# NTHU-LSALAB/KubeShare

Hardware: AMD Instinct MI355X
Metric: aggregate images/sec, co-located shared-GPU pods (higher is better)
Workload: dtype bf16; 1 GPU; model=resnet50, global_batch=512, image_size=224, parallelism=2 pods @ request=0.5, 2/GPU, pods_per_gpu=2, miopen_find=False, lease_accounting=sampled-busy

## Files before the change

kubeshare_amd/models/resnet.py:

```python
from __future__ import annotations

import torch
import torch.nn as nn

from .pool import FusedMaxPool2d


class Bottleneck(nn.Module):
    expansion = 4
    fused_ops = False

    def __init__(self, in_ch: int, width: int, stride: int = 1):
        super().__init__()
        out_ch = width * self.expansion
        self.conv1 = nn.Conv2d(in_ch, width, 1, bias=False)
        self.bn1 = nn.BatchNorm2d(width)
        self.conv2 = nn.Conv2d(width, width, 3, stride=stride, padding=1,
                               bias=False)
        self.bn2 = nn.BatchNorm2d(width)
        self.conv3 = nn.Conv2d(width, out_ch, 1, bias=False)
        self.bn3 = nn.BatchNorm2d(out_ch)
        self.relu = nn.ReLU(inplace=True)
        self.down = None
        if stride != 1 or in_ch != out_ch:
            self.down = nn.Sequential(
                nn.Conv2d(in_ch, out_ch, 1, stride=stride, bias=False),
                nn.BatchNorm2d(out_ch),
            )

    def forward(self, x):
        if self.fused_ops:
            from .. import ops
            identity = x if self.down is None else \
                ops.bn_relu(self.down[0](x), self.down[1], relu=False)
            out = ops.bn_relu(self.conv1(x), self.bn1)
            out = ops.bn_relu(self.conv2(out), self.bn2)
            return ops.bn_relu(self.conv3(out), self.bn3, res=identity)
        identity = x if self.down is None else self.down(x)
        out = self.relu(self.bn1(self.conv1(x)))
        out = self.relu(self.bn2(self.conv2(out)))
        out = self.bn3(self.conv3(out))
        return self.relu(out + identity)


class BasicBlock(nn.Module):
    expansion = 1
    fused_ops = False

    def __init__(self, in_ch: int, width: int, stride: int = 1):
        super().__init__()
        self.conv1 = nn.Conv2d(in_ch, width, 3, stride=stride, padding=1,
                               bias=False)
        self.bn1 = nn.BatchNorm2d(width)
        self.conv2 = nn.Conv2d(width, width, 3, padding=1, bias=False)
        self.bn2 = nn.BatchNorm2d(width)
        self.relu = nn.ReLU(inplace=True)
        self.down = None
        if stride != 1 or in_ch != width:
            self.down = nn.Sequential(
                nn.Conv2d(in_ch, width, 1, stride=stride, bias=False),
                nn.BatchNorm2d(width),
            )

    def forward(self, x):
        if self.fused_ops:
            from .. import ops
            identity = x if self.down is None else \
                ops.bn_relu(self.down[0](x), self.down[1], relu=False)
            out = ops.bn_relu(self.conv1(x), self.bn1)
            return ops.bn_relu(self.conv2(out), self.bn2, res=identity)
        identity = x if self.down is None else self.down(x)
        out = self.relu(self.bn1(self.conv1(x)))
        out = self.bn2(self.conv2(out))
        return self.relu(out + identity)


class ResNet(nn.Module):
    fused_ops = False

    def __init__(self, block, layers, num_classes: int = 1000):
        super().__init__()
        self.in_ch = 64
        self.conv1 = nn.Conv2d(3, 64, 7, stride=2, padding=3, bias=False)
        self.bn1 = nn.BatchNorm2d(64)
        self.relu = nn.ReLU(inplace=True)
        self.maxpool = FusedMaxPool2d(3, stride=2, padding=1)
        self.layer1 = self._make_layer(block, 64, layers[0])
        self.layer2 = self._make_layer(block, 128, layers[1], stride=2)
        self.layer3 = self._make_layer(block, 256, layers[2], stride=2)
        self.layer4 = self._make_layer(block, 512, layers[3], stride=2)
        self.avgpool = nn.AdaptiveAvgPool2d(1)
        self.fc = nn.Linear(512 * block.expansion, num_classes)
        for m in self.modules():
            if isinstance(m, nn.Conv2d):
                nn.init.kaiming_normal_(m.weight, mode="fan_out",
                                        nonlinearity="relu")
            elif isinstance(m, nn.BatchNorm2d):
                nn.init.ones_(m.weight)
                nn.init.zeros_(m.bias)

    def _make_layer(self, block, width, n, stride=1):
        layers = [block(self.in_ch, width, stride)]
        self.in_ch = width * block.expansion
        layers += [block(self.in_ch, width) for _ in range(n - 1)]
        return nn.Sequential(*layers)

    def forward(self, x):
        if self.fused_ops:
            from .. import ops
            x = self.maxpool(ops.bn_relu(self.conv1(x), self.bn1))
        else:
            x = self.maxpool(self.relu(self.bn1(self.conv1(x))))
        x = self.layer4(self.layer3(self.layer2(self.layer1(x))))
        x = torch.flatten(self.avgpool(x), 1)
        return self.fc(x)


def resnet18(num_classes: int = 1000) -> ResNet:
    return ResNet(BasicBlock, [2, 2, 2, 2], num_classes)


def resnet50(num_classes: int = 1000) -> ResNet:
    return ResNet(Bottleneck, [3, 4, 6, 3], num_classes)
```

kubeshare_amd/ops/__init__.py:

```python
from __future__ import annotations

import os

_HERE = os.path.dirname(os.path.abspath(__file__))
_BUILD_DIR = os.path.join(_HERE, "_build")
_SRCS = [os.path.join(_HERE, "hip", "ks_ops.hip"),
         os.path.join(_HERE, "hip", "bn_relu.hip"),
         os.path.join(_HERE, "hip", "pool.hip")]

_ext = None


def build_extension(verbose: bool = False):
    import torch
    from torch.utils import cpp_extension

    os.environ.setdefault("PYTORCH_ROCM_ARCH", "gfx950")
    os.makedirs(_BUILD_DIR, exist_ok=True)
    return cpp_extension.load(
        name="ks_ops",
        sources=_SRCS,
        build_directory=_BUILD_DIR,
        extra_cflags=["-O3"],
        verbose=verbose,
        is_python_module=True,
    )


def _load():
    global _ext
    if _ext is not None:
        return _ext
    import torch

    so = os.path.join(_BUILD_DIR, "ks_ops.so")
    if os.path.exists(so):
        import importlib.util

        spec = importlib.util.spec_from_file_location("ks_ops", so)
        mod = importlib.util.module_from_spec(spec)
        spec.loader.exec_module(mod)
        _ext = mod
        return _ext
    if torch.cuda.is_available():
        _ext = build_extension()
        return _ext
    raise ImportError(
        "kubeshare_amd.ops extension not built; run __graft_entry__.build()")


def burn(ms: float, blocks: int = 1024, threads: int = 256):
    _load().burn(float(ms), blocks, threads)


class FusedSGD:

    def __init__(self, params, lr: float, momentum: float = 0.9,
                 weight_decay: float = 0.0, graph_mode: str = "auto"):
        import torch

        self.params = [p for p in params if p.requires_grad]
        self.lr = lr
        self.momentum = momentum
        self.weight_decay = weight_decay
        self.momenta = [torch.zeros_like(p) for p in self.params]
        self._first = True
        self._graph_mode = graph_mode
        self._step_graph = None
        self._zero_graph = None
        self._graph_ptrs = None

    def _graphable(self):
        import torch
        if self._graph_mode == "off" or not torch.cuda.is_available():
            return False
        import os
        if os.environ.get("KUBESHARE_SGD_GRAPH", "1") == "0":
            return False
        return all(p.grad is not None and p.grad.is_cuda
                   for p in self.params)

    def zero_grad(self, set_to_none: bool = True):
        if self._zero_graph is not None and self._graph_ptrs == tuple(
                p.grad.data_ptr() if p.grad is not None else 0
                for p in self.params):
            self._zero_graph.replay()
            return
        for p in self.params:
            if p.grad is not None:
                if set_to_none and self._step_graph is None:
                    p.grad = None
                else:
                    p.grad.zero_()

    def _capture(self):
        import torch
        ext = _load()
        ps = [p.data for p in self.params]
        gs = [p.grad for p in self.params]
        vs = list(self.momenta)
        ptrs = tuple(g.data_ptr() for g in gs)
        step_g = torch.cuda.CUDAGraph()
        with torch.cuda.graph(step_g):
            ext.sgd_momentum_(ps, gs, vs, self.lr, self.momentum,
                              self.weight_decay)
        zero_g = torch.cuda.CUDAGraph()
        with torch.cuda.graph(zero_g):
            for g in gs:
                g.zero_()
        self._step_graph = step_g
        self._zero_graph = zero_g
        self._graph_ptrs = ptrs

    def step(self):
        ext = _load()
        if self._step_graph is not None and self._graph_ptrs == tuple(
                p.grad.data_ptr() if p.grad is not None else 0
                for p in self.params):
            self._step_graph.replay()
            return
        ps, gs, vs = [], [], []
        for p, v in zip(self.params, self.momenta):
            if p.grad is None:
                continue
            ps.append(p.data)
            gs.append(p.grad)
            vs.append(v)
        if self._first:
            self._first = False
        ext.sgd_momentum_(ps, gs, vs, self.lr, self.momentum,
                          self.weight_decay)
        if self._step_graph is None and self._graph_mode == "auto" and \
                len(gs) == len(self.params) and self._graphable():
            try:
                self._capture()
            except Exception:
                self._graph_mode = "off"


def _bn_relu_autograd():
    global _BNReLUFn
    if _BNReLUFn is not None:
        return _BNReLUFn
    import torch

    class BNReLUFn(torch.autograd.Function):

        @staticmethod
        def forward(ctx, x, res, weight, bias, running_mean, running_var,
                    training, momentum, eps, relu):
            ext = _load()
            w32 = weight.float()
            b32 = bias.float()
            if training:
                y, mean, invstd = ext.bn_relu_fwd_train(
                    x, w32, b32, running_mean, running_var, momentum, eps,
                    res, relu)
                ctx.save_for_backward(x, y, w32, b32, mean, invstd)
                ctx.with_res = res is not None
                ctx.relu = relu
                ctx.wdtype = weight.dtype
                return y
            y = ext.bn_relu_fwd_eval(x, w32, b32, running_mean.float(),
                                     running_var.float(), eps, res, relu)
            ctx.save_for_backward(x, y, w32, b32, running_mean.float(),
                                  (running_var.float() + eps).rsqrt())
            ctx.with_res = res is not None
            ctx.relu = relu
            ctx.wdtype = weight.dtype
            return y

        @staticmethod
        def backward(ctx, dy):
            ext = _load()
            x, y, w32, b32, mean, invstd = ctx.saved_tensors
            out = ext.bn_relu_bwd(x, y, dy, w32, b32, mean, invstd,
                                  ctx.with_res, ctx.relu)
            dx, dscale, dbias = out[0], out[1], out[2]
            dres = out[3] if ctx.with_res else None
            return (dx, dres, dscale.to(ctx.wdtype), dbias.to(ctx.wdtype),
                    None, None, None, None, None, None)

    _BNReLUFn = BNReLUFn
    return BNReLUFn


_BNReLUFn = None


def bn_relu(x, bn, res=None, relu=True):
    import torch

    supported = (x.dtype == torch.bfloat16 and x.size(1) % 8 == 0
                 and x.size(1) <= 2048 and x.is_cuda
                 and x.is_contiguous(memory_format=torch.channels_last))
    if supported and res is not None and res.dtype != torch.bfloat16:
        res = res.to(torch.bfloat16)
    if not supported:
        y = torch.nn.functional.batch_norm(
            x, bn.running_mean, bn.running_var, bn.weight, bn.bias,
            bn.training, bn.momentum, bn.eps)
        if res is not None:
            y = y + res
        return torch.relu(y) if relu else y
    if res is not None and not res.is_contiguous(
            memory_format=torch.channels_last):
        res = res.contiguous(memory_format=torch.channels_last)
    fn = _bn_relu_autograd()
    return fn.apply(x, res, bn.weight, bn.bias, bn.running_mean,
                    bn.running_var, bn.training, bn.momentum, bn.eps, relu)


_POOL_CONFIGS = ((3, 2, 1), (2, 2, 0))
_MaxPoolNHWCFn = None


def _pool_int(v):
    if type(v) is int:
        return v
    if isinstance(v, (tuple, list)) and len(v) == 2 and v[0] == v[1] \
            and type(v[0]) is int:
        return v[0]
    return None


def _pool_cfg(kernel_size, stride, padding):
    if stride is None or stride == () or stride == []:
        stride = kernel_size
    return (_pool_int(kernel_size), _pool_int(stride), _pool_int(padding))


def _pool_cfg_supported(x, cfg) -> bool:
    import torch

    if cfg not in _POOL_CONFIGS or x.dim() != 4:
        return False
    n, c, h, w = x.shape
    k, _, p = cfg
    return (x.is_cuda and x.dtype == torch.bfloat16
            and c % 8 == 0 and 8 <= c <= 2048 and n >= 1
            and h + 2 * p >= k and w + 2 * p >= k
            and n * h * w < 2 ** 31
            and x.is_contiguous(memory_format=torch.channels_last))


def fused_pool_enabled() -> bool:
    return os.environ.get("KUBESHARE_FUSED_POOL", "1") != "0"


def max_pool_supported(x, kernel_size, stride=None, padding=0) -> bool:
    return _pool_cfg_supported(x, _pool_cfg(kernel_size, stride, padding))


def _max_pool_autograd():
    global _MaxPoolNHWCFn
    if _MaxPoolNHWCFn is not None:
        return _MaxPoolNHWCFn
    import torch
    from torch.autograd.function import once_differentiable

    class MaxPoolNHWCFn(torch.autograd.Function):

        @staticmethod
        def forward(ctx, x, k, s, p, want_idx):
            out = _load().max_pool_nhwc_fwd(x, k, s, p, want_idx)
            if want_idx:
                ctx.save_for_backward(out[1])
                ctx.input_sizes = list(x.shape)
                ctx.cfg = (k, s, p)
            return out[0]

        @staticmethod
        @once_differentiable
        def backward(ctx, dy):
            (idx,) = ctx.saved_tensors
            if not dy.is_contiguous(memory_format=torch.channels_last):
                dy = dy.contiguous(memory_format=torch.channels_last)
            k, s, p = ctx.cfg
            dx = _load().max_pool_nhwc_bwd(dy, idx, ctx.input_sizes,
                                           k, s, p)
            return dx, None, None, None, None

    _MaxPoolNHWCFn = MaxPoolNHWCFn
    return MaxPoolNHWCFn


def max_pool_nhwc(x, kernel_size, stride=None, padding=0):
    import torch

    cfg = _pool_cfg(kernel_size, stride, padding)
    if not _pool_cfg_supported(x, cfg):
        return torch.nn.functional.max_pool2d(x, kernel_size, stride,
                                              padding)
# ... 12 lines not shown
```

kubeshare_amd/ops/hip/bn_relu.hip:

```cpp
#include <hip/hip_runtime.h>
#include <torch/extension.h>
#include <ATen/cuda/CUDAContext.h>

#include <vector>

typedef __attribute__((ext_vector_type(8))) unsigned short ushort8;
typedef __attribute__((ext_vector_type(8))) float float8;

__device__ __forceinline__ float bf16_to_f32(unsigned short u) {
  union {
    unsigned int i;
    float f;
  } v;
  v.i = ((unsigned int)u) << 16;
  return v.f;
}

__device__ __forceinline__ unsigned short f32_to_bf16(float f) {
  union {
    float f;
    unsigned int i;
  } v;
  v.f = f;
  unsigned int lsb = (v.i >> 16) & 1;
  v.i += 0x7fffu + lsb;
  return (unsigned short)(v.i >> 16);
}

#define KS_BN_BLOCK 512
#define KS_BN_UNROLL 4
#define KS_BN_UNROLL_STATS 8

__global__ void bn_stats_kernel(const ushort8* __restrict__ x,
                                float* __restrict__ part,
                                long long M, int CG) {
  __shared__ float s_red[KS_BN_BLOCK * 8];
  const int tid = threadIdx.x;
  const int cg = tid % CG;
  const int roff = tid / CG;
  const int rows_per_blk = KS_BN_BLOCK / CG;
  const bool active = roff < rows_per_blk;
  const long long stride = (long long)gridDim.x * rows_per_blk;

  float8 acc = {0, 0, 0, 0, 0, 0, 0, 0};
  float8 acc2 = {0, 0, 0, 0, 0, 0, 0, 0};
  long long row = active ? (long long)blockIdx.x * rows_per_blk + roff : M;
  for (; row + (KS_BN_UNROLL_STATS - 1) * stride < M;
       row += KS_BN_UNROLL_STATS * stride) {
    ushort8 v[KS_BN_UNROLL_STATS];
#pragma unroll
    for (int u = 0; u < KS_BN_UNROLL_STATS; u++)
      v[u] = x[(row + u * stride) * CG + cg];
#pragma unroll
    for (int u = 0; u < KS_BN_UNROLL_STATS; u++)
#pragma unroll
      for (int j = 0; j < 8; j++) {
        float f = bf16_to_f32(v[u][j]);
        acc[j] += f;
        acc2[j] += f * f;
      }
  }
  for (; row < M; row += stride) {
    ushort8 v = x[row * CG + cg];
#pragma unroll
    for (int j = 0; j < 8; j++) {
      float f = bf16_to_f32(v[j]);
      acc[j] += f;
      acc2[j] += f * f;
    }
  }

  const int C = CG * 8;
  float* sum_part = part + (long long)blockIdx.x * C;
  float* sq_part = part + (long long)(gridDim.x + blockIdx.x) * C;
#pragma unroll
  for (int j = 0; j < 8; j++) s_red[tid * 8 + j] = acc[j];
  __syncthreads();
  if (tid < CG) {
    float8 t = {0, 0, 0, 0, 0, 0, 0, 0};
    for (int r = 0; r < rows_per_blk; r++)
#pragma unroll
      for (int j = 0; j < 8; j++) t[j] += s_red[(r * CG + tid) * 8 + j];
#pragma unroll
    for (int j = 0; j < 8; j++) sum_part[tid * 8 + j] = t[j];
  }
  __syncthreads();
#pragma unroll
  for (int j = 0; j < 8; j++) s_red[tid * 8 + j] = acc2[j];
  __syncthreads();
  if (tid < CG) {
    float8 t = {0, 0, 0, 0, 0, 0, 0, 0};
    for (int r = 0; r < rows_per_blk; r++)
#pragma unroll
      for (int j = 0; j < 8; j++) t[j] += s_red[(r * CG + tid) * 8 + j];
#pragma unroll
    for (int j = 0; j < 8; j++) sq_part[tid * 8 + j] = t[j];
  }
}

__global__ void bn_reduce_partials_kernel(const float* __restrict__ part,
                                          int nblocks, int C,
                                          float* __restrict__ out0,
                                          float* __restrict__ out1) {
  const int lane = threadIdx.x;
  const int c = blockIdx.x * blockDim.y + threadIdx.y;
  if (c >= C) return;
  float a0 = 0.f, a1 = 0.f;
  for (int b = lane; b < nblocks; b += 64) {
    a0 += part[(long long)b * C + c];
    a1 += part[(long long)(nblocks + b) * C + c];
  }
#pragma unroll
  for (int off = 32; off > 0; off >>= 1) {
    a0 += __shfl_down(a0, off, 64);
// ... 12 lines not shown
                                   float* __restrict__ running_mean,
                                   float* __restrict__ running_var,
                                   float* __restrict__ save_mean,
                                   float* __restrict__ save_invstd,
                                   float* __restrict__ scale_out,
                                   float* __restrict__ bias_out,
                                   long long M, int C, float momentum,
                                   float eps) {
  int c = blockIdx.x * blockDim.x + threadIdx.x;
  if (c >= C) return;
  float mean = sum[c] / (float)M;
  float var = sumsq[c] / (float)M - mean * mean;
  var = var < 0.f ? 0.f : var;
  float invstd = rsqrtf(var + eps);
  save_mean[c] = mean;
  save_invstd[c] = invstd;
  if (running_mean) {
    float unbiased = M > 1 ? var * (float)M / (float)(M - 1) : var;
    running_mean[c] = (1.f - momentum) * running_mean[c] + momentum * mean;
    running_var[c] = (1.f - momentum) * running_var[c] + momentum * unbiased;
  }
  float s = weight[c] * invstd;
  scale_out[c] = s;
  bias_out[c] = bias[c] - mean * s;
}

template <bool WITH_RES, bool RELU = true>
__global__ void bn_apply_relu_kernel(const ushort8* __restrict__ x,
                                     const ushort8* __restrict__ res,
                                     ushort8* __restrict__ y,
                                     const float* __restrict__ scale,
                                     const float* __restrict__ biasf,
                                     long long M, int CG) {
  const int tid = threadIdx.x;
  const int cg = tid % CG;
  const int roff = tid / CG;
  const int rows_per_blk = KS_BN_BLOCK / CG;
  const bool active = roff < rows_per_blk;
  const long long stride = (long long)gridDim.x * rows_per_blk;
  float8 s, b;
#pragma unroll
  for (int j = 0; j < 8; j++) {
    s[j] = scale[cg * 8 + j];
    b[j] = biasf[cg * 8 + j];
  }
  long long row = active ? (long long)blockIdx.x * rows_per_blk + roff : M;
  for (; row + (KS_BN_UNROLL - 1) * stride < M;
       row += KS_BN_UNROLL * stride) {
    ushort8 v[KS_BN_UNROLL], r[KS_BN_UNROLL], o[KS_BN_UNROLL];
    long long k[KS_BN_UNROLL];
#pragma unroll
    for (int u = 0; u < KS_BN_UNROLL; u++) {
      k[u] = (row + u * stride) * CG + cg;
      v[u] = x[k[u]];
      if (WITH_RES) r[u] = res[k[u]];
    }
#pragma unroll
    for (int u = 0; u < KS_BN_UNROLL; u++) {
#pragma unroll
      for (int j = 0; j < 8; j++) {
        float f = fmaf(bf16_to_f32(v[u][j]), s[j], b[j]);
        if (WITH_RES) f += bf16_to_f32(r[u][j]);
        o[u][j] = f32_to_bf16(RELU && f < 0.f ? 0.f : f);
      }
      y[k[u]] = o[u];
    }
  }
  for (; row < M; row += stride) {
    const long long k = row * CG + cg;
    ushort8 v = x[k];
    ushort8 r;
    if (WITH_RES) r = res[k];
    ushort8 o;
#pragma unroll
    for (int j = 0; j < 8; j++) {
      float f = fmaf(bf16_to_f32(v[j]), s[j], b[j]);
      if (WITH_RES) f += bf16_to_f32(r[j]);
      o[j] = f32_to_bf16(RELU && f < 0.f ? 0.f : f);
    }
    y[k] = o;
  }
}

template <bool WRITE_DYM>
__global__ void bn_bwd_stats_kernel(const ushort8* __restrict__ x,
                                    const ushort8* __restrict__ y,
                                    const ushort8* __restrict__ dy,
                                    ushort8* __restrict__ dym_out,
                                    const float* __restrict__ mean,
                                    const float* __restrict__ invstd,
                                    float* __restrict__ part,
                                    long long M, int CG) {
  __shared__ float s_red[KS_BN_BLOCK * 8];
  const int tid = threadIdx.x;
  const int cg = tid % CG;
  const int roff = tid / CG;
  const int rows_per_blk = KS_BN_BLOCK / CG;
  const bool active = roff < rows_per_blk;
  const long long stride = (long long)gridDim.x * rows_per_blk;
  float8 mu, is;
#pragma unroll
  for (int j = 0; j < 8; j++) {
    mu[j] = mean[cg * 8 + j];
    is[j] = invstd[cg * 8 + j];
  }
  float8 adb = {0, 0, 0, 0, 0, 0, 0, 0};
  float8 ads = {0, 0, 0, 0, 0, 0, 0, 0};
  long long row = active ? (long long)blockIdx.x * rows_per_blk + roff : M;
  for (; row + (KS_BN_UNROLL - 1) * stride < M;
       row += KS_BN_UNROLL * stride) {
    ushort8 xv[KS_BN_UNROLL], yv[KS_BN_UNROLL], gv[KS_BN_UNROLL];
    long long k[KS_BN_UNROLL];
#pragma unroll
    for (int u = 0; u < KS_BN_UNROLL; u++) {
      k[u] = (row + u * stride) * CG + cg;
      xv[u] = x[k[u]];
      yv[u] = y[k[u]];
      gv[u] = dy[k[u]];
    }
#pragma unroll
    for (int u = 0; u < KS_BN_UNROLL; u++) {
      ushort8 dm;
#pragma unroll
      for (int j = 0; j < 8; j++) {
        float g = bf16_to_f32(yv[u][j]) > 0.f ? bf16_to_f32(gv[u][j]) : 0.f;
        float xhat = (bf16_to_f32(xv[u][j]) - mu[j]) * is[j];
        adb[j] += g;
        ads[j] += g * xhat;
        if (WRITE_DYM) dm[j] = f32_to_bf16(g);
      }
      if (WRITE_DYM) dym_out[k[u]] = dm;
    }
  }
  for (; row < M; row += stride) {
    const long long k = row * CG + cg;
    ushort8 xv = x[k], yv = y[k], gv = dy[k];
    ushort8 dm;
#pragma unroll
    for (int j = 0; j < 8; j++) {
      float g = bf16_to_f32(yv[j]) > 0.f ? bf16_to_f32(gv[j]) : 0.f;
      float xhat = (bf16_to_f32(xv[j]) - mu[j]) * is[j];
      adb[j] += g;
      ads[j] += g * xhat;
      if (WRITE_DYM) dm[j] = f32_to_bf16(g);
    }
    if (WRITE_DYM) dym_out[k] = dm;
  }

  const int C = CG * 8;
  float* db_part = part + (long long)blockIdx.x * C;
  float* ds_part = part + (long long)(gridDim.x + blockIdx.x) * C;
#pragma unroll
  for (int j = 0; j < 8; j++) s_red[tid * 8 + j] = adb[j];
  __syncthreads();
  if (tid < CG) {
    float8 t = {0, 0, 0, 0, 0, 0, 0, 0};
    for (int r = 0; r < rows_per_blk; r++)
#pragma unroll
      for (int j = 0; j < 8; j++) t[j] += s_red[(r * CG + tid) * 8 + j];
#pragma unroll
    for (int j = 0; j < 8; j++) db_part[tid * 8 + j] = t[j];
  }
  __syncthreads();
#pragma unroll
  for (int j = 0; j < 8; j++) s_red[tid * 8 + j] = ads[j];
  __syncthreads();
  if (tid < CG) {
    float8 t = {0, 0, 0, 0, 0, 0, 0, 0};
    for (int r = 0; r < rows_per_blk; r++)
#pragma unroll
      for (int j = 0; j < 8; j++) t[j] += s_red[(r * CG + tid) * 8 + j];
#pragma unroll
    for (int j = 0; j < 8; j++) ds_part[tid * 8 + j] = t[j];
  }
}

template <bool RELU = true>
__global__ void bn_bwd_stats_noy_kernel(const ushort8* __restrict__ x,
                                        const ushort8* __restrict__ dy,
                                        const float* __restrict__ mean,
                                        const float* __restrict__ invstd,
                                        const float* __restrict__ weight,
                                        const float* __restrict__ bias,
                                        float* __restrict__ part,
                                        long long M, int CG) {
  __shared__ float s_red[KS_BN_BLOCK * 8];
  const int tid = threadIdx.x;
  const int cg = tid % CG;
  const int roff = tid / CG;
  const int rows_per_blk = KS_BN_BLOCK / CG;
  const bool active = roff < rows_per_blk;
  const long long stride = (long long)gridDim.x * rows_per_blk;
  float8 mu, is, sc, bf;
#pragma unroll
  for (int j = 0; j < 8; j++) {
    const int c = cg * 8 + j;
    mu[j] = mean[c];
    is[j] = invstd[c];
    sc[j] = weight[c] * is[j];
    bf[j] = bias[c] - mu[j] * sc[j];
  }
  float8 adb = {0, 0, 0, 0, 0, 0, 0, 0};
  float8 ads = {0, 0, 0, 0, 0, 0, 0, 0};
  long long row = active ? (long long)blockIdx.x * rows_per_blk + roff : M;
  for (; row + (KS_BN_UNROLL - 1) * stride < M;
       row += KS_BN_UNROLL * stride) {
    ushort8 xv[KS_BN_UNROLL], gv[KS_BN_UNROLL];
#pragma unroll
    for (int u = 0; u < KS_BN_UNROLL; u++) {
      const long long k = (row + u * stride) * CG + cg;
      xv[u] = x[k];
      gv[u] = dy[k];
    }
#pragma unroll
    for (int u = 0; u < KS_BN_UNROLL; u++)
#pragma unroll
      for (int j = 0; j < 8; j++) {
        float xf = bf16_to_f32(xv[u][j]);
        float g = bf16_to_f32(gv[u][j]);
        if (RELU) {
          float f = fmaf(xf, sc[j], bf[j]);
          if (!f32_to_bf16(f > 0.f ? f : 0.f)) g = 0.f;
        }
        adb[j] += g;
        ads[j] += g * ((xf - mu[j]) * is[j]);
      }
// ... 305 lines not shown
  auto sums = at::empty({2 * g.C}, f32);

  hipLaunchKernelGGL(bn_stats_kernel, dim3(g.stat_blocks),
                     dim3(KS_BN_BLOCK), 0, stream.stream(),
                     reinterpret_cast<const ushort8*>(x.data_ptr()),
                     part.data_ptr<float>(), g.M, g.CG);
  hipLaunchKernelGGL(bn_reduce_partials_kernel,
                     dim3((g.C + 3) / 4), dim3(64, 4), 0, stream.stream(),
                     part.data_ptr<float>(), g.stat_blocks, g.C,
                     sums.data_ptr<float>(), sums.data_ptr<float>() + g.C);
  int fb = (g.C + 255) / 256;
  hipLaunchKernelGGL(bn_finalize_kernel, dim3(fb), dim3(256), 0,
                     stream.stream(), sums.data_ptr<float>(),
                     sums.data_ptr<float>() + g.C,
                     weight.data_ptr<float>(), bias.data_ptr<float>(),
                     running_mean.defined()
                         ? running_mean.data_ptr<float>() : nullptr,
                     running_var.defined()
                         ? running_var.data_ptr<float>() : nullptr,
                     save_mean.data_ptr<float>(),
                     save_invstd.data_ptr<float>(), scale.data_ptr<float>(),
                     biasf.data_ptr<float>(), g.M, g.C, (float)momentum,
                     (float)eps);
  auto launch_apply = [&](auto kern) {
    hipLaunchKernelGGL(kern, dim3(g.blocks), dim3(KS_BN_BLOCK), 0,
                       stream.stream(),
                       reinterpret_cast<const ushort8*>(x.data_ptr()),
                       res.has_value()
                           ? reinterpret_cast<const ushort8*>(res->data_ptr())
                           : nullptr,
                       reinterpret_cast<ushort8*>(y.data_ptr()),
                       scale.data_ptr<float>(), biasf.data_ptr<float>(), g.M,
                       g.CG);
  };
  if (res.has_value())
    relu ? launch_apply(bn_apply_relu_kernel<true, true>)
         : launch_apply(bn_apply_relu_kernel<true, false>);
  else
    relu ? launch_apply(bn_apply_relu_kernel<false, true>)
         : launch_apply(bn_apply_relu_kernel<false, false>);
  return {y, save_mean, save_invstd};
}

torch::Tensor bn_relu_fwd_eval(torch::Tensor x, torch::Tensor weight,
                               torch::Tensor bias, torch::Tensor rmean,
                               torch::Tensor rvar, double eps,
                               c10::optional<torch::Tensor> res, bool relu) {
  Geom g = geom_of(x);
  auto stream = at::cuda::getCurrentCUDAStream();
  auto f32 = x.options().dtype(at::kFloat);
  auto scale = at::empty({g.C}, f32);
  auto biasf = at::empty({g.C}, f32);
  auto y = at::empty_like(x);
  int fb = (g.C + 255) / 256;
  hipLaunchKernelGGL(bn_fold_eval_kernel, dim3(fb), dim3(256), 0,
                     stream.stream(), weight.data_ptr<float>(),
                     bias.data_ptr<float>(), rmean.data_ptr<float>(),
                     rvar.data_ptr<float>(), scale.data_ptr<float>(),
                     biasf.data_ptr<float>(), g.C, (float)eps);
  auto launch_apply = [&](auto kern) {
    hipLaunchKernelGGL(kern, dim3(g.blocks), dim3(KS_BN_BLOCK), 0,
                       stream.stream(),
                       reinterpret_cast<const ushort8*>(x.data_ptr()),
                       res.has_value()
                           ? reinterpret_cast<const ushort8*>(res->data_ptr())
                           : nullptr,
                       reinterpret_cast<ushort8*>(y.data_ptr()),
                       scale.data_ptr<float>(), biasf.data_ptr<float>(), g.M,
                       g.CG);
  };
  if (res.has_value())
    relu ? launch_apply(bn_apply_relu_kernel<true, true>)
         : launch_apply(bn_apply_relu_kernel<true, false>);
  else
    relu ? launch_apply(bn_apply_relu_kernel<false, true>)
         : launch_apply(bn_apply_relu_kernel<false, false>);
  return y;
}

std::vector<torch::Tensor> bn_relu_bwd(torch::Tensor x, torch::Tensor y,
                                       torch::Tensor dy, torch::Tensor weight,
                                       torch::Tensor bias, torch::Tensor mean,
                                       torch::Tensor invstd, bool need_dres,
                                       bool relu) {
  TORCH_CHECK(relu || !need_dres,
              "bn_relu_bwd: residual path requires the ReLU variant");
  Geom g = geom_of(x);
  auto stream = at::cuda::getCurrentCUDAStream();
  auto f32 = x.options().dtype(at::kFloat);
  auto part = at::empty({(long long)2 * g.stat_blocks * g.C}, f32);
  auto red = at::empty({g.C * 2}, f32);
  float* dbias_p = red.data_ptr<float>();
  float* dscale_p = dbias_p + g.C;
  auto dx = at::empty_like(x);
  torch::Tensor dres;
  if (!dy.is_contiguous(at::MemoryFormat::ChannelsLast))
    dy = dy.contiguous(at::MemoryFormat::ChannelsLast);

  if (need_dres) {
    dres = at::empty_like(x);
    hipLaunchKernelGGL(bn_bwd_stats_kernel<true>, dim3(g.stat_blocks),
                       dim3(KS_BN_BLOCK), 0, stream.stream(),
                       reinterpret_cast<const ushort8*>(x.data_ptr()),
                       reinterpret_cast<const ushort8*>(y.data_ptr()),
                       reinterpret_cast<const ushort8*>(dy.data_ptr()),
                       reinterpret_cast<ushort8*>(dres.data_ptr()),
                       mean.data_ptr<float>(), invstd.data_ptr<float>(),
                       part.data_ptr<float>(), g.M, g.CG);
    hipLaunchKernelGGL(bn_reduce_partials_kernel,
                       dim3((g.C + 3) / 4), dim3(64, 4), 0, stream.stream(),
                       part.data_ptr<float>(), g.stat_blocks, g.C,
                       dbias_p, dscale_p);
    hipLaunchKernelGGL(bn_bwd_apply_dym_kernel, dim3(g.blocks),
                       dim3(KS_BN_BLOCK), 0, stream.stream(),
                       reinterpret_cast<const ushort8*>(x.data_ptr()),
                       reinterpret_cast<const ushort8*>(dres.data_ptr()),
                       reinterpret_cast<ushort8*>(dx.data_ptr()),
                       mean.data_ptr<float>(), invstd.data_ptr<float>(),
                       weight.data_ptr<float>(), dbias_p, dscale_p,
                       g.M, g.CG);
    auto dbias = red.narrow(0, 0, g.C);
    auto dscale = red.narrow(0, g.C, g.C);
    return {dx, dscale, dbias, dres};
  }
  auto launch_stats = [&](auto kern) {
    hipLaunchKernelGGL(kern, dim3(g.stat_blocks), dim3(KS_BN_BLOCK), 0,
                       stream.stream(),
                       reinterpret_cast<const ushort8*>(x.data_ptr()),
                       reinterpret_cast<const ushort8*>(dy.data_ptr()),
                       mean.data_ptr<float>(), invstd.data_ptr<float>(),
                       weight.data_ptr<float>(), bias.data_ptr<float>(),
                       part.data_ptr<float>(), g.M, g.CG);
  };
  relu ? launch_stats(bn_bwd_stats_noy_kernel<true>)
       : launch_stats(bn_bwd_stats_noy_kernel<false>);
  hipLaunchKernelGGL(bn_reduce_partials_kernel,
                     dim3((g.C + 3) / 4), dim3(64, 4), 0, stream.stream(),
                     part.data_ptr<float>(), g.stat_blocks, g.C,
                     dbias_p, dscale_p);
  auto launch_bapply = [&](auto kern) {
    hipLaunchKernelGGL(kern, dim3(g.blocks), dim3(KS_BN_BLOCK), 0,
                       stream.stream(),
                       reinterpret_cast<const ushort8*>(x.data_ptr()),
                       reinterpret_cast<const ushort8*>(dy.data_ptr()),
                       reinterpret_cast<ushort8*>(dx.data_ptr()),
                       mean.data_ptr<float>(), invstd.data_ptr<float>(),
                       weight.data_ptr<float>(), bias.data_ptr<float>(),
                       dbias_p, dscale_p, g.M, g.CG);
  };
  relu ? launch_bapply(bn_bwd_apply_noy_kernel<true>)
       : launch_bapply(bn_bwd_apply_noy_kernel<false>);
  auto dbias = red.narrow(0, 0, g.C);
  auto dscale = red.narrow(0, g.C, g.C);
  return {dx, dscale, dbias};
}
```

kubeshare_amd/ops/hip/ks_ops.hip:

```cpp
#include <hip/hip_runtime.h>
#include <torch/extension.h>
#include <ATen/cuda/CUDAContext.h>

#include <vector>

#define WAVE 64

__global__ void burn_kernel(long long ticks, float* sink) {
  long long start = wall_clock64();
  float acc = threadIdx.x * 1e-9f;
  while (wall_clock64() - start < ticks) {
#pragma unroll
    for (int i = 0; i < 64; i++) acc = fmaf(acc, 1.0000001f, 1e-12f);
  }
  if (acc == 12345.678f) sink[0] = acc;
}

void burn(double ms, int64_t blocks, int64_t threads) {
  long long ticks = (long long)(ms * 100000.0);
  auto stream = at::cuda::getCurrentCUDAStream();
  static float* sink = nullptr;
  if (!sink) {
    if (hipMalloc(&sink, sizeof(float)) != hipSuccess)
      throw std::runtime_error("burn: hipMalloc failed");
  }
  hipLaunchKernelGGL(burn_kernel, dim3((uint32_t)blocks),
                     dim3((uint32_t)threads), 0, stream.stream(), ticks,
                     sink);
}

template <typename T>
struct Vec4;
template <>
struct Vec4<float> {
  using type = float4;
};

__global__ void sgd_mom_f32_kernel(float* __restrict__ p,
                                   const float* __restrict__ g,
                                   float* __restrict__ v, float lr, float mu,
                                   float wd, long long n) {
  long long i = (long long)blockIdx.x * blockDim.x + threadIdx.x;
  long long stride = (long long)gridDim.x * blockDim.x;
  long long n4 = n / 4;
  const float4* g4 = reinterpret_cast<const float4*>(g);
  float4* p4 = reinterpret_cast<float4*>(p);
  float4* v4 = reinterpret_cast<float4*>(v);
  for (long long k = i; k < n4; k += stride) {
    float4 pv = p4[k], gv = g4[k], vv = v4[k];
    vv.x = mu * vv.x + gv.x + wd * pv.x;
    vv.y = mu * vv.y + gv.y + wd * pv.y;
    vv.z = mu * vv.z + gv.z + wd * pv.z;
    vv.w = mu * vv.w + gv.w + wd * pv.w;
    pv.x -= lr * vv.x;
    pv.y -= lr * vv.y;
    pv.z -= lr * vv.z;
    pv.w -= lr * vv.w;
    v4[k] = vv;
    p4[k] = pv;
  }
  for (long long k = n4 * 4 + i; k < n; k += stride) {
    float vv = mu * v[k] + g[k] + wd * p[k];
    v[k] = vv;
    p[k] -= lr * vv;
  }
}

void sgd_momentum_(std::vector<torch::Tensor> params,
                   std::vector<torch::Tensor> grads,
                   std::vector<torch::Tensor> momenta, double lr, double mu,
                   double wd) {
  auto stream = at::cuda::getCurrentCUDAStream();
  for (size_t t = 0; t < params.size(); t++) {
    auto& p = params[t];
    auto& g = grads[t];
    auto& v = momenta[t];
    TORCH_CHECK(p.is_cuda() && p.scalar_type() == at::kFloat &&
                    p.is_non_overlapping_and_dense() &&
                    g.sizes() == p.sizes() && g.strides() == p.strides() &&
                    v.strides() == p.strides() &&
                    g.scalar_type() == at::kFloat &&
                    v.scalar_type() == at::kFloat,
                "sgd_momentum_: f32 dense tensors with matching strides "
                "(any memory format: the update is elementwise over the "
                "flat storage)");
    long long n = p.numel();
    int threads = 256;
    int blocks = (int)std::min<long long>(2048, (n / 4 + threads - 1) / threads + 1);
    hipLaunchKernelGGL(sgd_mom_f32_kernel, dim3(blocks), dim3(threads), 0,
                       stream.stream(), p.data_ptr<float>(),
                       g.data_ptr<float>(), v.data_ptr<float>(), (float)lr,
                       (float)mu, (float)wd, n);
  }
}

std::vector<torch::Tensor> bn_relu_fwd_train(
    torch::Tensor x, torch::Tensor weight, torch::Tensor bias,
    torch::Tensor running_mean, torch::Tensor running_var, double momentum,
    double eps, c10::optional<torch::Tensor> res, bool relu);
torch::Tensor bn_relu_fwd_eval(torch::Tensor x, torch::Tensor weight,
                               torch::Tensor bias, torch::Tensor rmean,
                               torch::Tensor rvar, double eps,
                               c10::optional<torch::Tensor> res, bool relu);
std::vector<torch::Tensor> bn_relu_bwd(torch::Tensor x, torch::Tensor y,
                                       torch::Tensor dy, torch::Tensor weight,
                                       torch::Tensor bias, torch::Tensor mean,
                                       torch::Tensor invstd, bool need_dres,
                                       bool relu);

std::vector<torch::Tensor> max_pool_nhwc_fwd(torch::Tensor x, int64_t k,
                                             int64_t s, int64_t p,
                                             bool want_idx);
torch::Tensor max_pool_nhwc_bwd(torch::Tensor dy, torch::Tensor idx,
                                std::vector<int64_t> input_sizes, int64_t k,
                                int64_t s, int64_t p);

PYBIND11_MODULE(TORCH_EXTENSION_NAME, m) {
  m.def("burn", &burn, "occupy the GPU for ~ms milliseconds",
        py::arg("ms"), py::arg("blocks") = 1024, py::arg("threads") = 256);
  m.def("sgd_momentum_", &sgd_momentum_,
        "fused SGD+momentum update (in-place)");
  m.def("bn_relu_fwd_train", &bn_relu_fwd_train);
  m.def("bn_relu_fwd_eval", &bn_relu_fwd_eval);
  m.def("bn_relu_bwd", &bn_relu_bwd);
  m.def("max_pool_nhwc_fwd", &max_pool_nhwc_fwd);
  m.def("max_pool_nhwc_bwd", &max_pool_nhwc_bwd);
}
```

Measured before the change: 8231 images/s.

## Fork residual outputs to fold gradient sums into BN backward; multi-tensor SGD

Each residual block now returns its output as a pair, one copy for the main path and one for the identity path. The two incoming gradients are then added inside the BN-ReLU backward stats kernel, which avoids autograd materialising a separate gradient-accumulation add. The SGD momentum update is replaced by a multi-tensor kernel that packs many parameters into a few launches, and the optimizer no longer captures a zero-grad graph. The cost is extra complexity in the autograd function and a change to the dscale accumulation rounding, since some channels now use an unfused multiply-add.

```diff
diff --git a/kubeshare_amd/models/resnet.py b/kubeshare_amd/models/resnet.py
--- a/kubeshare_amd/models/resnet.py
+++ b/kubeshare_amd/models/resnet.py
@@ -29,18 +29,22 @@
             )
 
     def forward(self, x):
+        pair = isinstance(x, tuple)
+        x, x_id = x if pair else (x, x)
         if self.fused_ops:
             from .. import ops
-            identity = x if self.down is None else \
-                ops.bn_relu(self.down[0](x), self.down[1], relu=False)
+            identity = x_id if self.down is None else \
+                ops.bn_relu(self.down[0](x_id), self.down[1], relu=False)
             out = ops.bn_relu(self.conv1(x), self.bn1)
             out = ops.bn_relu(self.conv2(out), self.bn2)
-            return ops.bn_relu(self.conv3(out), self.bn3, res=identity)
-        identity = x if self.down is None else self.down(x)
+            return ops.bn_relu(self.conv3(out), self.bn3, res=identity,
+                               fork=pair)
+        identity = x_id if self.down is None else self.down(x_id)
         out = self.relu(self.bn1(self.conv1(x)))
         out = self.relu(self.bn2(self.conv2(out)))
         out = self.bn3(self.conv3(out))
-        return self.relu(out + identity)
+        out = self.relu(out + identity)
+        return (out, out) if pair else out
 
 
 class BasicBlock(nn.Module):
@@ -63,16 +67,20 @@
             )
 
     def forward(self, x):
+        pair = isinstance(x, tuple)
+        x, x_id = x if pair else (x, x)
         if self.fused_ops:
             from .. import ops
-            identity = x if self.down is None else \
-                ops.bn_relu(self.down[0](x), self.down[1], relu=False)
+            identity = x_id if self.down is None else \
+                ops.bn_relu(self.down[0](x_id), self.down[1], relu=False)
             out = ops.bn_relu(self.conv1(x), self.bn1)
-            return ops.bn_relu(self.conv2(out), self.bn2, res=identity)
-        identity = x if self.down is None else self.down(x)
+            return ops.bn_relu(self.conv2(out), self.bn2, res=identity,
+                               fork=pair)
+        identity = x_id if self.down is None else self.down(x_id)
         out = self.relu(self.bn1(self.conv1(x)))
         out = self.bn2(self.conv2(out))
-        return self.relu(out + identity)
+        out = self.relu(out + identity)
+        return (out, out) if pair else out
 
 
 class ResNet(nn.Module):
@@ -109,9 +117,13 @@
         if self.fused_ops:
             from .. import ops
             x = self.maxpool(ops.bn_relu(self.conv1(x), self.bn1))
+            if ops.bn_fork_enabled():
+                x = (x, x)
         else:
             x = self.maxpool(self.relu(self.bn1(self.conv1(x))))
         x = self.layer4(self.layer3(self.layer2(self.layer1(x))))
+        if isinstance(x, tuple):
+            x = x[0]
         x = torch.flatten(self.avgpool(x), 1)
         return self.fc(x)
 
diff --git a/kubeshare_amd/ops/__init__.py b/kubeshare_amd/ops/__init__.py
--- a/kubeshare_amd/ops/__init__.py
+++ b/kubeshare_amd/ops/__init__.py
@@ -64,60 +64,40 @@
         self.momentum = momentum
         self.weight_decay = weight_decay
         self.momenta = [torch.zeros_like(p) for p in self.params]
-        self._first = True
         self._graph_mode = graph_mode
+        self._multi = os.environ.get("KUBESHARE_SGD_MULTI", "1") != "0"
         self._step_graph = None
-        self._zero_graph = None
         self._graph_ptrs = None
 
     def _graphable(self):
         import torch
         if self._graph_mode == "off" or not torch.cuda.is_available():
             return False
-        import os
         if os.environ.get("KUBESHARE_SGD_GRAPH", "1") == "0":
             return False
         return all(p.grad is not None and p.grad.is_cuda
                    for p in self.params)
 
+    def _ptrs(self):
+        return tuple(
+            (p.data_ptr(), v.data_ptr(),
+             p.grad.data_ptr() if p.grad is not None else 0)
+            for p, v in zip(self.params, self.momenta))
+
     def zero_grad(self, set_to_none: bool = True):
-        if self._zero_graph is not None and self._graph_ptrs == tuple(
-                p.grad.data_ptr() if p.grad is not None else 0
-                for p in self.params):
-            self._zero_graph.replay()
-            return
         for p in self.params:
-            if p.grad is not None:
-                if set_to_none and self._step_graph is None:
-                    p.grad = None
-                else:
-                    p.grad.zero_()
-
-    def _capture(self):
-        import torch
+            if set_to_none:
+                p.grad = None
+            elif p.grad is not None:
+                p.grad.zero_()
+
+    def _launch(self):
         ext = _load()
-        ps = [p.data for p in self.params]
-        gs = [p.grad for p in self.params]
-        vs = list(self.momenta)
-        ptrs = tuple(g.data_ptr() for g in gs)
-        step_g = torch.cuda.CUDAGraph()
-        with torch.cuda.graph(step_g):
-            ext.sgd_momentum_(ps, gs, vs, self.lr, self.momentum,
-                              self.weight_decay)
-        zero_g = torch.cuda.CUDAGraph()
-        with torch.cuda.graph(zero_g):
-            for g in gs:
-                g.zero_()
-        self._step_graph = step_g
-        self._zero_graph = zero_g
-        self._graph_ptrs = ptrs
-
-    def step(self):
-        ext = _load()
-        if self._step_graph is not None and self._graph_ptrs == tuple(
-                p.grad.data_ptr() if p.grad is not None else 0
-                for p in self.params):
-            self._step_graph.replay()
+        if self._multi:
+            ext.sgd_momentum_multi_(
+                [p.data for p in self.params],
+                [p.grad for p in self.params], self.momenta,
+                self.lr, self.momentum, self.weight_decay)
             return
         ps, gs, vs = [], [], []
         for p, v in zip(self.params, self.momenta):
@@ -126,12 +106,26 @@
             ps.append(p.data)
             gs.append(p.grad)
             vs.append(v)
-        if self._first:
-            self._first = False
         ext.sgd_momentum_(ps, gs, vs, self.lr, self.momentum,
                           self.weight_decay)
+
+    def _capture(self):
+        import torch
+        ptrs = self._ptrs()
+        step_g = torch.cuda.CUDAGraph()
+        with torch.cuda.graph(step_g):
+            self._launch()
+        self._step_graph = step_g
+        self._graph_ptrs = ptrs
+
+    def step(self):
+        if self._step_graph is not None and \
+                self._graph_ptrs == self._ptrs():
+            self._step_graph.replay()
+            return
+        self._launch()
         if self._step_graph is None and self._graph_mode == "auto" and \
-                len(gs) == len(self.params) and self._graphable():
+                self._graphable():
             try:
                 self._capture()
             except Exception:
@@ -148,38 +142,40 @@
 
         @staticmethod
         def forward(ctx, x, res, weight, bias, running_mean, running_var,
-                    training, momentum, eps, relu):
+                    training, momentum, eps, relu, fork=False):
             ext = _load()
             w32 = weight.float()
             b32 = bias.float()
+            ctx.set_materialize_grads(False)
+            ctx.with_res = res is not None
+            ctx.relu = relu
+            ctx.wdtype = weight.dtype
             if training:
                 y, mean, invstd = ext.bn_relu_fwd_train(
                     x, w32, b32, running_mean, running_var, momentum, eps,
                     res, relu)
                 ctx.save_for_backward(x, y, w32, b32, mean, invstd)
-                ctx.with_res = res is not None
-                ctx.relu = relu
-                ctx.wdtype = weight.dtype
-                return y
-            y = ext.bn_relu_fwd_eval(x, w32, b32, running_mean.float(),
-                                     running_var.float(), eps, res, relu)
-            ctx.save_for_backward(x, y, w32, b32, running_mean.float(),
-                                  (running_var.float() + eps).rsqrt())
-            ctx.with_res = res is not None
-            ctx.relu = relu
-            ctx.wdtype = weight.dtype
-            return y
+            else:
+                y = ext.bn_relu_fwd_eval(x, w32, b32, running_mean.float(),
+                                         running_var.float(), eps, res, relu)
+                ctx.save_for_backward(x, y, w32, b32, running_mean.float(),
+                                      (running_var.float() + eps).rsqrt())
+            return (y, y.view_as(y)) if fork else y
 
         @staticmethod
-        def backward(ctx, dy):
+        def backward(ctx, dy, dy2=None):
             ext = _load()
             x, y, w32, b32, mean, invstd = ctx.saved_tensors
+            if dy is None:
+                dy, dy2 = dy2, None
+            if dy is None:
+                return (None,) * 11
             out = ext.bn_relu_bwd(x, y, dy, w32, b32, mean, invstd,
-                                  ctx.with_res, ctx.relu)
+                                  ctx.with_res, ctx.relu, dy2)
             dx, dscale, dbias = out[0], out[1], out[2]
             dres = out[3] if ctx.with_res else None
             return (dx, dres, dscale.to(ctx.wdtype), dbias.to(ctx.wdtype),
-                    None, None, None, None, None, None)
+                    None, None, None, None, None, None, None)
 
     _BNReLUFn = BNReLUFn
     return BNReLUFn
@@ -188,7 +184,11 @@
 _BNReLUFn = None
 
 
-def bn_relu(x, bn, res=None, relu=True):
+def bn_fork_enabled() -> bool:
+    return os.environ.get("KUBESHARE_BN_FORK", "1") != "0"
+
+
+def bn_relu(x, bn, res=None, relu=True, fork=False):
     import torch
 
     supported = (x.dtype == torch.bfloat16 and x.size(1) % 8 == 0
@@ -202,13 +202,15 @@
             bn.training, bn.momentum, bn.eps)
         if res is not None:
             y = y + res
-        return torch.relu(y) if relu else y
+        y = torch.relu(y) if relu else y
+        return (y, y) if fork else y
     if res is not None and not res.is_contiguous(
             memory_format=torch.channels_last):
         res = res.contiguous(memory_format=torch.channels_last)
     fn = _bn_relu_autograd()
     return fn.apply(x, res, bn.weight, bn.bias, bn.running_mean,
-                    bn.running_var, bn.training, bn.momentum, bn.eps, relu)
+                    bn.running_var, bn.training, bn.momentum, bn.eps, relu,
+                    fork)
 
 
 _POOL_CONFIGS = ((3, 2, 1), (2, 2, 0))
diff --git a/kubeshare_amd/ops/hip/bn_relu.hip b/kubeshare_amd/ops/hip/bn_relu.hip
--- a/kubeshare_amd/ops/hip/bn_relu.hip
+++ b/kubeshare_amd/ops/hip/bn_relu.hip
@@ -30,6 +30,7 @@
 #define KS_BN_BLOCK 512
 #define KS_BN_UNROLL 4
 #define KS_BN_UNROLL_STATS 8
+#define KS_BN_UNROLL_DY2 2
 
 __global__ void bn_stats_kernel(const ushort8* __restrict__ x,
                                 float* __restrict__ part,
@@ -208,10 +209,30 @@
   }
 }
 
-template <bool WRITE_DYM>
+__device__ __forceinline__ float bn_join_grad(unsigned short a,
+                                              unsigned short b) {
+  return bf16_to_f32(f32_to_bf16(bf16_to_f32(a) + bf16_to_f32(b)));
+}
+
+__device__ __forceinline__ float bn_mul_add_unfused(float acc, float a,
+                                                    float b) {
+#pragma clang fp contract(off)
+  float prod = a * b;
+  return acc + prod;
+}
+
+template <bool GROUPED>
+__device__ __forceinline__ float bn_acc_dscale(float acc, float g, float xhat,
+                                               int j) {
+  return (GROUPED && j >= 6) ? bn_mul_add_unfused(acc, g, xhat)
+                             : fmaf(g, xhat, acc);
+}
+
+template <bool WRITE_DYM, bool WITH_DY2 = false>
 __global__ void bn_bwd_stats_kernel(const ushort8* __restrict__ x,
                                     const ushort8* __restrict__ y,
                                     const ushort8* __restrict__ dy,
+                                    const ushort8* __restrict__ dy2,
                                     ushort8* __restrict__ dym_out,
                                     const float* __restrict__ mean,
                                     const float* __restrict__ invstd,
@@ -232,42 +253,54 @@
   }
   float8 adb = {0, 0, 0, 0, 0, 0, 0, 0};
   float8 ads = {0, 0, 0, 0, 0, 0, 0, 0};
+  constexpr int U = WITH_DY2 ? KS_BN_UNROLL_DY2 : KS_BN_UNROLL;
+  static_assert(KS_BN_UNROLL % U == 0, "sub-batches must tile a group");
   long long row = active ? (long long)blockIdx.x * rows_per_blk + roff : M;
   for (; row + (KS_BN_UNROLL - 1) * stride < M;
        row += KS_BN_UNROLL * stride) {
-    ushort8 xv[KS_BN_UNROLL], yv[KS_BN_UNROLL], gv[KS_BN_UNROLL];
-    long long k[KS_BN_UNROLL];
-#pragma unroll
-    for (int u = 0; u < KS_BN_UNROLL; u++) {
-      k[u] = (row + u * stride) * CG + cg;
-      xv[u] = x[k[u]];
-      yv[u] = y[k[u]];
-      gv[u] = dy[k[u]];
-    }
-#pragma unroll
-    for (int u = 0; u < KS_BN_UNROLL; u++) {
-      ushort8 dm;
-#pragma unroll
-      for (int j = 0; j < 8; j++) {
-        float g = bf16_to_f32(yv[u][j]) > 0.f ? bf16_to_f32(gv[u][j]) : 0.f;
-        float xhat = (bf16_to_f32(xv[u][j]) - mu[j]) * is[j];
-        adb[j] += g;
-        ads[j] += g * xhat;
-        if (WRITE_DYM) dm[j] = f32_to_bf16(g);
-      }
-      if (WRITE_DYM) dym_out[k[u]] = dm;
+#pragma unroll 1
+    for (int h = 0; h < KS_BN_UNROLL; h += U) {
+      ushort8 xv[U], yv[U], gv[U];
+      ushort8 g2[U];
+      long long k[U];
+#pragma unroll
+      for (int u = 0; u < U; u++) {
+        k[u] = (row + (h + u) * stride) * CG + cg;
+        xv[u] = x[k[u]];
+        yv[u] = y[k[u]];
+        gv[u] = dy[k[u]];
+        if (WITH_DY2) g2[u] = dy2[k[u]];
+      }
+#pragma unroll
+      for (int u = 0; u < U; u++) {
+        ushort8 dm;
+#pragma unroll
+        for (int j = 0; j < 8; j++) {
+          float gin = WITH_DY2 ? bn_join_grad(gv[u][j], g2[u][j])
+                               : bf16_to_f32(gv[u][j]);
+          float g = bf16_to_f32(yv[u][j]) > 0.f ? gin : 0.f;
+          float xhat = (bf16_to_f32(xv[u][j]) - mu[j]) * is[j];
+          adb[j] += g;
+          ads[j] = bn_acc_dscale<true>(ads[j], g, xhat, j);
+          if (WRITE_DYM) dm[j] = f32_to_bf16(g);
+        }
+        if (WRITE_DYM) dym_out[k[u]] = dm;
+      }
     }
   }
   for (; row < M; row += stride) {
     const long long k = row * CG + cg;
     ushort8 xv = x[k], yv = y[k], gv = dy[k];
+    ushort8 g2;
+    if (WITH_DY2) g2 = dy2[k];
     ushort8 dm;
 #pragma unroll
     for (int j = 0; j < 8; j++) {
-      float g = bf16_to_f32(yv[j]) > 0.f ? bf16_to_f32(gv[j]) : 0.f;
+      float gin = WITH_DY2 ? bn_join_grad(gv[j], g2[j]) : bf16_to_f32(gv[j]);
+      float g = bf16_to_f32(yv[j]) > 0.f ? gin : 0.f;
       float xhat = (bf16_to_f32(xv[j]) - mu[j]) * is[j];
       adb[j] += g;
-      ads[j] += g * xhat;
+      ads[j] = bn_acc_dscale<false>(ads[j], g, xhat, j);
       if (WRITE_DYM) dm[j] = f32_to_bf16(g);
     }
     if (WRITE_DYM) dym_out[k] = dm;
@@ -739,10 +772,24 @@
                                        torch::Tensor dy, torch::Tensor weight,
                                        torch::Tensor bias, torch::Tensor mean,
                                        torch::Tensor invstd, bool need_dres,
-                                       bool relu) {
+                                       bool relu,
+                                       c10::optional<torch::Tensor> dy2) {
   TORCH_CHECK(relu || !need_dres,
               "bn_relu_bwd: residual path requires the ReLU variant");
   Geom g = geom_of(x);
+  TORCH_CHECK(dy.sizes() == x.sizes() && y.sizes() == x.sizes() &&
+                  dy.scalar_type() == at::kBFloat16,
+              "bn_relu_bwd: dy must be bf16 of x's shape");
+  bool fold_dy2 = false;
+  if (dy2.has_value() && dy2->defined()) {
+    TORCH_CHECK(dy2->sizes() == x.sizes(),
+                "bn_relu_bwd: dy2 must have x's shape");
+    fold_dy2 = need_dres && dy2->is_cuda() &&
+               dy2->scalar_type() == at::kBFloat16 &&
+               dy2->is_contiguous(at::MemoryFormat::ChannelsLast) &&
+               dy.is_contiguous(at::MemoryFormat::ChannelsLast);
+    if (!fold_dy2) dy = (dy + *dy2).to(at::kBFloat16);
+  }
   auto stream = at::cuda::getCurrentCUDAStream();
   auto f32 = x.options().dtype(at::kFloat);
   auto part = at::empty({(long long)2 * g.stat_blocks * g.C}, f32);
@@ -756,14 +803,21 @@
 
   if (need_dres) {
     dres = at::empty_like(x);
-    hipLaunchKernelGGL(bn_bwd_stats_kernel<true>, dim3(g.stat_blocks),
-                       dim3(KS_BN_BLOCK), 0, stream.stream(),
-                       reinterpret_cast<const ushort8*>(x.data_ptr()),
-                       reinterpret_cast<const ushort8*>(y.data_ptr()),
-                       reinterpret_cast<const ushort8*>(dy.data_ptr()),
-                       reinterpret_cast<ushort8*>(dres.data_ptr()),
-                       mean.data_ptr<float>(), invstd.data_ptr<float>(),
-                       part.data_ptr<float>(), g.M, g.CG);
+    auto launch_rstats = [&](auto kern) {
+      hipLaunchKernelGGL(kern, dim3(g.stat_blocks), dim3(KS_BN_BLOCK), 0,
+                         stream.stream(),
+                         reinterpret_cast<const ushort8*>(x.data_ptr()),
+                         reinterpret_cast<const ushort8*>(y.data_ptr()),
+                         reinterpret_cast<const ushort8*>(dy.data_ptr()),
+                         fold_dy2 ? reinterpret_cast<const ushort8*>(
+                                        dy2->data_ptr())
+                                  : nullptr,
+                         reinterpret_cast<ushort8*>(dres.data_ptr()),
+                         mean.data_ptr<float>(), invstd.data_ptr<float>(),
+                         part.data_ptr<float>(), g.M, g.CG);
+    };
+    fold_dy2 ? launch_rstats(bn_bwd_stats_kernel<true, true>)
+             : launch_rstats(bn_bwd_stats_kernel<true, false>);
     hipLaunchKernelGGL(bn_reduce_partials_kernel,
                        dim3((g.C + 3) / 4), dim3(64, 4), 0, stream.stream(),
                        part.data_ptr<float>(), g.stat_blocks, g.C,
diff --git a/kubeshare_amd/ops/hip/ks_ops.hip b/kubeshare_amd/ops/hip/ks_ops.hip
--- a/kubeshare_amd/ops/hip/ks_ops.hip
+++ b/kubeshare_amd/ops/hip/ks_ops.hip
@@ -35,6 +35,21 @@
 struct Vec4<float> {
   using type = float4;
 };
+
+__device__ __forceinline__ void sgd_mom_update(float& p, float g, float& v,
+                                               float lr, float mu, float wd) {
+  v = fmaf(wd, p, fmaf(mu, v, g));
+  p = fmaf(-lr, v, p);
+}
+
+__device__ __forceinline__ void sgd_mom_update4(float4& p, const float4& g,
+                                                float4& v, float lr, float mu,
+                                                float wd) {
+  sgd_mom_update(p.x, g.x, v.x, lr, mu, wd);
+  sgd_mom_update(p.y, g.y, v.y, lr, mu, wd);
+  sgd_mom_update(p.z, g.z, v.z, lr, mu, wd);
+  sgd_mom_update(p.w, g.w, v.w, lr, mu, wd);
+}
 
 __global__ void sgd_mom_f32_kernel(float* __restrict__ p,
                                    const float* __restrict__ g,
@@ -48,21 +63,98 @@
   float4* v4 = reinterpret_cast<float4*>(v);
   for (long long k = i; k < n4; k += stride) {
     float4 pv = p4[k], gv = g4[k], vv = v4[k];
-    vv.x = mu * vv.x + gv.x + wd * pv.x;
-    vv.y = mu * vv.y + gv.y + wd * pv.y;
-    vv.z = mu * vv.z + gv.z + wd * pv.z;
-    vv.w = mu * vv.w + gv.w + wd * pv.w;
-    pv.x -= lr * vv.x;
-    pv.y -= lr * vv.y;
-    pv.z -= lr * vv.z;
-    pv.w -= lr * vv.w;
+    sgd_mom_update4(pv, gv, vv, lr, mu, wd);
     v4[k] = vv;
     p4[k] = pv;
   }
   for (long long k = n4 * 4 + i; k < n; k += stride) {
-    float vv = mu * v[k] + g[k] + wd * p[k];
+    float pv = p[k], vv = v[k];
+    sgd_mom_update(pv, g[k], vv, lr, mu, wd);
     v[k] = vv;
-    p[k] -= lr * vv;
+    p[k] = pv;
+  }
+}
+
+#define KS_SGD_THREADS 256
+#define KS_SGD_VPT 4
+#define KS_SGD_CHUNK (KS_SGD_THREADS * KS_SGD_VPT * 4)
+#define KS_SGD_MAX_TENSORS 110
+
+struct SgdMultiArgs {
+  float* p[KS_SGD_MAX_TENSORS];
+  const float* g[KS_SGD_MAX_TENSORS];
+  float* v[KS_SGD_MAX_TENSORS];
+  long long n[KS_SGD_MAX_TENSORS];
+  int blk[KS_SGD_MAX_TENSORS + 1];
+  int count;
+  float lr, mu, wd;
+};
+static_assert(sizeof(SgdMultiArgs) <= 4096,
+              "SgdMultiArgs must fit the 4 KiB kernel-argument segment");
+
+__global__ void __launch_bounds__(KS_SGD_THREADS)
+sgd_mom_multi_f32_kernel(const SgdMultiArgs a) {
+  const int b = blockIdx.x;
+  int lo = 0, hi = a.count - 1;
+  while (lo < hi) {
+    int mid = (lo + hi + 1) >> 1;
+    if (a.blk[mid] <= b) lo = mid; else hi = mid - 1;
+  }
+  float* __restrict__ p = a.p[lo];
+  const float* __restrict__ g = a.g[lo];
+  float* __restrict__ v = a.v[lo];
+  const long long n = a.n[lo];
+  const float lr = a.lr, mu = a.mu, wd = a.wd;
+  const long long base = (long long)(b - a.blk[lo]) * KS_SGD_CHUNK;
+  long long rem = n - base;
+  const int len = rem < KS_SGD_CHUNK ? (int)rem : KS_SGD_CHUNK;
+  p += base;
+  g += base;
+  v += base;
+  const int tid = threadIdx.x;
+  const bool vec = (((uintptr_t)p | (uintptr_t)g | (uintptr_t)v) & 15) == 0;
+  if (vec) {
+    const int len4 = len >> 2;
+    const float4* g4 = reinterpret_cast<const float4*>(g);
+    float4* p4 = reinterpret_cast<float4*>(p);
+    float4* v4 = reinterpret_cast<float4*>(v);
+    if (len == KS_SGD_CHUNK) {
+      float4 pv[KS_SGD_VPT], gv[KS_SGD_VPT], vv[KS_SGD_VPT];
+#pragma unroll
+      for (int u = 0; u < KS_SGD_VPT; u++) {
+        const int k = tid + u * KS_SGD_THREADS;
+        pv[u] = p4[k];
+        gv[u] = g4[k];
+        vv[u] = v4[k];
+      }
+#pragma unroll
+      for (int u = 0; u < KS_SGD_VPT; u++) {
+        const int k = tid + u * KS_SGD_THREADS;
+        sgd_mom_update4(pv[u], gv[u], vv[u], lr, mu, wd);
+        v4[k] = vv[u];
+        p4[k] = pv[u];
+      }
+      return;
+    }
+    for (int k = tid; k < len4; k += KS_SGD_THREADS) {
+      float4 pv = p4[k], gv = g4[k], vv = v4[k];
+      sgd_mom_update4(pv, gv, vv, lr, mu, wd);
+      v4[k] = vv;
+      p4[k] = pv;
+    }
+    for (int k = len4 * 4 + tid; k < len; k += KS_SGD_THREADS) {
+      float pv = p[k], vv = v[k];
+      sgd_mom_update(pv, g[k], vv, lr, mu, wd);
+      v[k] = vv;
+      p[k] = pv;
+    }
+    return;
+  }
+  for (int k = tid; k < len; k += KS_SGD_THREADS) {
+    float pv = p[k], vv = v[k];
+    sgd_mom_update(pv, g[k], vv, lr, mu, wd);
+    v[k] = vv;
+    p[k] = pv;
   }
 }
 
@@ -94,6 +186,76 @@
   }
 }
 
+int64_t sgd_momentum_multi_(std::vector<torch::Tensor> params,
+                            std::vector<c10::optional<torch::Tensor>> grads,
+                            std::vector<torch::Tensor> momenta, double lr,
+                            double mu, double wd) {
+  TORCH_CHECK(params.size() == grads.size() &&
+                  params.size() == momenta.size(),
+              "sgd_momentum_multi_: params, grads and momenta differ in "
+              "length");
+  auto stream = at::cuda::getCurrentCUDAStream();
+  const long long max_blocks = 1LL << 30;
+  SgdMultiArgs a = {};
+  a.lr = (float)lr;
+  a.mu = (float)mu;
+  a.wd = (float)wd;
+  a.count = 0;
+  a.blk[0] = 0;
+  int64_t launches = 0;
+  std::vector<torch::Tensor> keep;
+  auto flush = [&]() {
+    if (a.count == 0) return;
+    hipLaunchKernelGGL(sgd_mom_multi_f32_kernel, dim3(a.blk[a.count]),
+                       dim3(KS_SGD_THREADS), 0, stream.stream(), a);
+    launches++;
+    a.count = 0;
+  };
+  for (size_t t = 0; t < params.size(); t++) {
+    if (!grads[t].has_value() || !grads[t]->defined()) continue;
+    auto& p = params[t];
+    auto& v = momenta[t];
+    torch::Tensor g = *grads[t];
+    TORCH_CHECK(g.sizes() == p.sizes() && g.is_cuda() &&
+                    g.scalar_type() == at::kFloat,
+                "sgd_momentum_multi_: f32 CUDA gradient of the "
+                "parameter's shape expected");
+    if (g.strides() != p.strides()) {
+      g = at::empty_like(p).copy_(g);
+      keep.push_back(g);
+    }
+    TORCH_CHECK(p.is_cuda() && p.scalar_type() == at::kFloat &&
+                    p.is_non_overlapping_and_dense() &&
+                    g.sizes() == p.sizes() && g.strides() == p.strides() &&
+                    v.strides() == p.strides() &&
+                    g.scalar_type() == at::kFloat &&
+                    v.scalar_type() == at::kFloat,
+                "sgd_momentum_: f32 dense tensors with matching strides "
+                "(any memory format: the update is elementwise over the "
+                "flat storage)");
+    TORCH_CHECK(v.is_cuda() && v.sizes() == p.sizes() &&
+                    p.get_device() == stream.device_index() &&
+                    g.get_device() == p.get_device() &&
+                    v.get_device() == p.get_device(),
+                "sgd_momentum_multi_: parameter, gradient and momentum "
+                "must live on the current device and share a shape");
+    const long long n = p.numel();
+    if (n == 0) continue;
+    const long long nb = (n + KS_SGD_CHUNK - 1) / KS_SGD_CHUNK;
+    TORCH_CHECK(nb <= max_blocks, "sgd_momentum_multi_: tensor too large");
+    if (a.count == KS_SGD_MAX_TENSORS || a.blk[a.count] + nb > max_blocks)
+      flush();
+    a.p[a.count] = p.data_ptr<float>();
+    a.g[a.count] = g.data_ptr<float>();
+    a.v[a.count] = v.data_ptr<float>();
+    a.n[a.count] = n;
+    a.blk[a.count + 1] = a.blk[a.count] + (int)nb;
+    a.count++;
+  }
+  flush();
+  return launches;
+}
+
 std::vector<torch::Tensor> bn_relu_fwd_train(
     torch::Tensor x, torch::Tensor weight, torch::Tensor bias,
     torch::Tensor running_mean, torch::Tensor running_var, double momentum,
@@ -106,7 +268,8 @@
                                        torch::Tensor dy, torch::Tensor weight,
                                        torch::Tensor bias, torch::Tensor mean,
                                        torch::Tensor invstd, bool need_dres,
-                                       bool relu);
+                                       bool relu,
+                                       c10::optional<torch::Tensor> dy2);
 
 std::vector<torch::Tensor> max_pool_nhwc_fwd(torch::Tensor x, int64_t k,
                                              int64_t s, int64_t p,
@@ -120,9 +283,16 @@
         py::arg("ms"), py::arg("blocks") = 1024, py::arg("threads") = 256);
   m.def("sgd_momentum_", &sgd_momentum_,
         "fused SGD+momentum update (in-place)");
+  m.def("sgd_momentum_multi_", &sgd_momentum_multi_,
+        "fused SGD+momentum update of all tensors in as few launches as "
+        "the kernel-argument limit allows; a None gradient skips its "
+        "tensor; returns the number of launches");
   m.def("bn_relu_fwd_train", &bn_relu_fwd_train);
   m.def("bn_relu_fwd_eval", &bn_relu_fwd_eval);
-  m.def("bn_relu_bwd", &bn_relu_bwd);
+  m.def("bn_relu_bwd", &bn_relu_bwd, py::arg("x"), py::arg("y"),
+        py::arg("dy"), py::arg("weight"), py::arg("bias"), py::arg("mean"),
+        py::arg("invstd"), py::arg("need_dres"), py::arg("relu"),
+        py::arg("dy2") = py::none());
   m.def("max_pool_nhwc_fwd", &max_pool_nhwc_fwd);
   m.def("max_pool_nhwc_bwd", &max_pool_nhwc_bwd);
 }
```

Result: faster. 8800 images/s, median of 6 (+6.9%).
